# avianphysics/avian

Hardware: AMD Instinct MI355X
Metric: physics substeps/sec at N dynamic bodies (3D) (higher is better)
Workload: dtype f32; 1 GPU; cfg2_box_stack_100k; dynamic_bodies_per_gpu=100000, manifolds_per_gpu=678200, contact_points_per_gpu=2712800, broadphase_pairs=1244836, substeps=4, hip_graph=True, narrow_phase=out of path: fixed synthetic face manifolds

## Files before the change

### avian_amd/csrc/k_contacts.hip

```cpp
#include <cstdlib>

#include "avn_kernels.h"
#include "avn_body_ops.h"

namespace avn {

#define CONTACT_THREADS 64

template <class T> struct BodyRef {
    V3<T> v, om, dp;
    Q4<T> dq;
    V3<T> inv_mass;
    Sym3<T> I;
    T lin_w, ang_w;
};

template <class T> struct BodyView { Vec4<T> *lin, *ang, *dp, *dq, *sia, *sib; };
template <class T> __device__ __forceinline__ BodyView<T> global_bodies(const DW<T>& w) { return {w.sb_lin.p, w.sb_ang.p, w.sb_dp.p, w.sb_dq.p, w.si_a.p, w.si_b.p}; }

typedef uint32_t u32x4 __attribute__((ext_vector_type(4)));
#define AVN_BUF_AUX_SC1 16
template <class V> __device__ __forceinline__ __amdgpu_buffer_rsrc_t rec_rsrc(V* base) { return __builtin_amdgcn_make_buffer_rsrc((void*)base, 0, 0x7FFFFFFF, 0x00020000); }
__device__ __forceinline__ Vec4<float> ld_rec_agent(Vec4<float>* base, size_t idx) {
    const u32x4 r = __builtin_amdgcn_raw_buffer_load_b128(rec_rsrc(base), (int)(idx * sizeof(Vec4<float>)), 0, AVN_BUF_AUX_SC1);
    return make4<float>(__uint_as_float(r.x), __uint_as_float(r.y), __uint_as_float(r.z), __uint_as_float(r.w));
}
__device__ __forceinline__ Vec4<double> ld_rec_agent(Vec4<double>* base, size_t idx) {
    const __amdgpu_buffer_rsrc_t rs = rec_rsrc(base);
    const u32x4 a = __builtin_amdgcn_raw_buffer_load_b128(rs, (int)(idx * sizeof(Vec4<double>)), 0, AVN_BUF_AUX_SC1);
    const u32x4 b = __builtin_amdgcn_raw_buffer_load_b128(rs, (int)(idx * sizeof(Vec4<double>) + 16), 0, AVN_BUF_AUX_SC1);
    return make4<double>(__hiloint2double((int)a.y, (int)a.x), __hiloint2double((int)a.w, (int)a.z), __hiloint2double((int)b.y, (int)b.x), __hiloint2double((int)b.w, (int)b.z));
}
__device__ __forceinline__ void st_rec_agent(Vec4<float>* base, size_t idx, Vec4<float> v) {
    __builtin_amdgcn_raw_buffer_store_b128(u32x4{__float_as_uint(v.x), __float_as_uint(v.y), __float_as_uint(v.z), __float_as_uint(v.w)}, rec_rsrc(base), (int)(idx * sizeof(Vec4<float>)), 0,
                                           AVN_BUF_AUX_SC1);
}
__device__ __forceinline__ void st_rec_agent(Vec4<double>* base, size_t idx, Vec4<double> v) {
    const __amdgpu_buffer_rsrc_t rs = rec_rsrc(base);
    __builtin_amdgcn_raw_buffer_store_b128(u32x4{(uint32_t)__double2loint(v.x), (uint32_t)__double2hiint(v.x), (uint32_t)__double2loint(v.y), (uint32_t)__double2hiint(v.y)}, rs,
                                           (int)(idx * sizeof(Vec4<double>)), 0, AVN_BUF_AUX_SC1);
    __builtin_amdgcn_raw_buffer_store_b128(u32x4{(uint32_t)__double2loint(v.z), (uint32_t)__double2hiint(v.z), (uint32_t)__double2loint(v.w), (uint32_t)__double2hiint(v.w)}, rs,
                                           (int)(idx * sizeof(Vec4<double>) + 16), 0, AVN_BUF_AUX_SC1);
}
template <class T, bool WITH_DELTA> __device__ __forceinline__ void body_from_recs(Vec4<T> l, Vec4<T> a, Vec4<T> dp, Vec4<T> dq, Vec4<T> sa, Vec4<T> sb, bool no_body, bool dummy_inertia, BodyRef<T>& b) {
    const T z = T(0);
    b.v = V3<T>{no_body ? z : l.x, no_body ? z : l.y, no_body ? z : l.z};
    b.om = V3<T>{no_body ? z : a.x, no_body ? z : a.y, no_body ? z : a.z};
    b.lin_w = no_body ? z : l.w; b.ang_w = no_body ? z : a.w;
    const bool nd = no_body || !WITH_DELTA;
    b.dp = V3<T>{nd ? z : dp.x, nd ? z : dp.y, nd ? z : dp.z};
    b.dq = Q4<T>{nd ? z : dq.x, nd ? z : dq.y, nd ? z : dq.z, nd ? T(1) : dq.w};
    const bool ni = no_body || dummy_inertia;
    V3<T> em = effective_inv_mass<T>(sa.x, scalar_to_bits(sb.w));
    b.inv_mass = V3<T>{ni ? z : em.x, ni ? z : em.y, ni ? z : em.z};
    b.I = Sym3<T>{ni ? z : sa.y, ni ? z : sa.z, ni ? z : sa.w, ni ? z : sb.x, ni ? z : sb.y, ni ? z : sb.z};
}
template <class T, bool WITH_DELTA, int STRIDE, bool COH = false>
__device__ __forceinline__ void load_body(const BodyView<T>& bv, int idx, bool no_body, bool dummy_inertia, BodyRef<T>& b) {
    const size_t o = (size_t)idx * STRIDE;
    Vec4<T> l, a;
    if (COH) { l = ld_rec_agent(bv.lin, o); a = ld_rec_agent(bv.ang, o); }
    else { l = bv.lin[o]; a = bv.ang[o]; }
    Vec4<T> dp = make4<T>(0, 0, 0, 0), dq = make4<T>(0, 0, 0, 1);
    if (WITH_DELTA) { dp = bv.dp[o]; dq = bv.dq[o]; }
    Vec4<T> sa = bv.sia[o], sb = bv.sib[o];
    body_from_recs<T, WITH_DELTA>(l, a, dp, dq, sa, sb, no_body, dummy_inertia, b);
}
template <class T, int STRIDE, bool COH = false> __device__ __forceinline__ void store_body(const BodyView<T>& bv, int idx, bool no_body, const BodyRef<T>& b) {
    if (no_body) return;
    if (COH) { st_rec_agent(bv.lin, (size_t)idx * STRIDE, make4<T>(b.v, b.lin_w)); st_rec_agent(bv.ang, (size_t)idx * STRIDE, make4<T>(b.om, b.ang_w)); return; }
    bv.lin[(size_t)idx * STRIDE] = make4<T>(b.v, b.lin_w);
// ... 301 lines not shown
        contributions(r, ent, true, dl);
#pragma unroll
        for (uint32_t k = 0; k < AVN_MAX_MANIFOLD_POINTS; ++k) { v.x = v.x + dl.d[k][0]; v.y = v.y + dl.d[k][1]; v.z = v.z + dl.d[k][2]; om.x = om.x + dl.d[k][3]; om.y = om.y + dl.d[k][4]; om.z = om.z + dl.d[k][5]; }
    }
    const uint32_t n_ent = (uint32_t)__popc(mask);
    uint32_t rest = mask;
    for (uint32_t j0 = 0; j0 < n_ent; j0 += 4u) {
        uint32_t mine = rest;
        for (uint32_t t = 0; t < q; ++t) mine &= mine - 1u;
        const bool present = mine != 0u;
        const uint32_t c = present ? (uint32_t)__ffs((int)mine) - 1u : 0u;
        rest &= rest - 1u; rest &= rest - 1u; rest &= rest - 1u; rest &= rest - 1u;
        const uint32_t sc = present ? w.inc_slot[(size_t)c * w.inc_stride + body] : 0u;
        WarmRecords<T> r; QuadDelta<T> dl;
        warm_fetch<T>(w, sc, r);
        contributions(r, sc, present, dl);
        quad_accumulate<0, T>(dl, v, om); quad_accumulate<1, T>(dl, v, om); quad_accumulate<2, T>(dl, v, om); quad_accumulate<3, T>(dl, v, om);
    }
    if (q == 0u) {
        w.sb_lin[body] = make4<T>(v, l4.w);
        w.sb_ang[body] = make4<T>(om, a4.w);
    }
}

template <class T, int STRIDE>
__device__ __forceinline__ void warm_core(const DW<T>& w, const StepParams<T>& p, uint32_t m, const BodyView<T>& bv, int i1, int i2) {
    Vec4<T> h1 = w.c_h1[m], h0 = w.m_n[m];
    const uint32_t S = w.m_stride;
    Vec4<T> pa[AVN_MAX_MANIFOLD_POINTS], pb[AVN_MAX_MANIFOLD_POINTS], pd[AVN_MAX_MANIFOLD_POINTS];
#pragma unroll
    for (uint32_t k = 0; k < AVN_MAX_MANIFOLD_POINTS; ++k) { uint32_t s = k * S + m; pa[k] = w.c_pa[s]; pb[k] = w.c_pb[s]; pd[k] = w.c_pd[s]; }
    const uint32_t cm = scalar_to_bits(h1.w);
    const uint32_t np = cm & 7u;
    BodyRef<T> b1, b2;
    load_body<T, false, STRIDE>(bv, i1, cm & AVN_CM_NOBODY1, cm & AVN_CM_DOM1, b1);
    load_body<T, false, STRIDE>(bv, i2, cm & AVN_CM_NOBODY2, cm & AVN_CM_DOM2, b2);
    if (np == 0) return;
    const V3<T> normal = xyz<T>(h0);
    const V3<T> t0 = xyz<T>(h1), t1 = cross(t0, normal);
    const T coeff = p.warm_start_coefficient;
#pragma unroll
    for (uint32_t k = 0; k < AVN_MAX_MANIFOLD_POINTS; ++k) {
        if (k < np) {
            const Vec4<T> d = pd[k];
            const T tx = (cm & AVN_CM_TANGENT) ? d.z : T(0), ty = (cm & AVN_CM_TANGENT) ? d.w : T(0);
            const V3<T> imp = coeff * ((d.x * normal + tx * t0) + ty * t1);
            apply_impulse(b1, b2, imp, xyz<T>(pa[k]), xyz<T>(pb[k]));
        }
    }
    store_body<T, STRIDE>(bv, i1, cm & AVN_CM_NOBODY1, b1);
    store_body<T, STRIDE>(bv, i2, cm & AVN_CM_NOBODY2, b2);
}

template <class T, bool USE_BIAS, int STRIDE, bool COH = false>
__device__ __forceinline__ void solve_core(const DW<T>& w, const StepParams<T>& p, uint32_t m, const BodyView<T>& bv, int i1, int i2) {
    Vec4<T> h1 = w.c_h1[m];
    Vec4<T> h0 = w.m_n[m];
    Vec4<T> h2 = w.m_tv[m];
    uint32_t S = w.m_stride;
    Vec4<T> pa[AVN_MAX_MANIFOLD_POINTS], pb[AVN_MAX_MANIFOLD_POINTS], pc[AVN_MAX_MANIFOLD_POINTS], pd[AVN_MAX_MANIFOLD_POINTS];
#pragma unroll
    for (uint32_t k = 0; k < AVN_MAX_MANIFOLD_POINTS; ++k) {
        uint32_t s = k * S + m;
        pa[k] = w.c_pa[s]; pb[k] = w.c_pb[s]; pc[k] = w.c_pc[s]; pd[k] = w.c_pd[s];
    }
    uint32_t cm = scalar_to_bits(h1.w);
    uint32_t np = cm & 7u;
    BodyRef<T> b1, b2;
    load_body<T, true, STRIDE, COH>(bv, i1, cm & AVN_CM_NOBODY1, cm & AVN_CM_DOM1, b1);
    load_body<T, true, STRIDE, COH>(bv, i2, cm & AVN_CM_NOBODY2, cm & AVN_CM_DOM2, b2);
    if (np == 0) return;
    V3<T> normal = xyz<T>(h0);
    T friction = h0.w;
    SoftCoef<T> soft = (cm & AVN_CM_SOFT_ND) ? p.soft_non_dynamic : p.soft_dynamic;
    T delta_secs = p.h_adj;
    V3<T> delta_translation = b2.dp - b1.dp;
#pragma unroll
    for (uint32_t k = 0; k < AVN_MAX_MANIFOLD_POINTS; ++k) {
        if (k < np) {
            V3<T> a1 = xyz<T>(pa[k]), a2 = xyz<T>(pb[k]);
            V3<T> r1w = qrot(b1.dq, a1), r2w = qrot(b2.dq, a2);
            V3<T> delta_separation = delta_translation + (r2w - r1w);
            T separation = dot(delta_separation, normal) + pa[k].w;
            V3<T> relative_velocity = velocity_at_point(b2, a2) - velocity_at_point(b1, a1);
            T normal_speed = dot(relative_velocity, normal);
            T eff_mass = pb[k].w, acc = pd[k].x;
            T impulse;
            if (separation > T(0)) {
                impulse = -eff_mass * (normal_speed + separation / delta_secs);
            } else if (USE_BIAS) {
                T bias = smax(soft.bias * separation, -p.max_overlap_solve_speed);
                T scaled_mass = soft.mass_scale * eff_mass;
                T scaled_impulse = soft.impulse_scale * acc;
                impulse = -scaled_mass * (normal_speed + bias) - scaled_impulse;
            } else {
                impulse = -eff_mass * normal_speed;
            }
            T new_impulse = smax(acc + impulse, T(0));
            impulse = new_impulse - acc;
            pd[k].x = new_impulse;
            pd[k].y = pd[k].y + new_impulse;
            apply_impulse(b1, b2, impulse * normal, a1, a2);
        }
    }
    if (cm & AVN_CM_TANGENT) {
        V3<T> t0 = xyz<T>(h1), t1 = cross(t0, normal);
        V3<T> surface_velocity = xyz<T>(h2);
#pragma unroll
        for (uint32_t k = 0; k < AVN_MAX_MANIFOLD_POINTS; ++k) {
            if (k < np) {
                V3<T> a1 = xyz<T>(pa[k]), a2 = xyz<T>(pb[k]);
                V3<T> relative_velocity = velocity_at_point(b2, a2) - velocity_at_point(b1, a1);
                T impulse_limit = friction * pd[k].x;
                V3<T> rv = relative_velocity + surface_velocity;
                T ts1 = dot(rv, t0), ts2 = dot(rv, t1);
                T t11 = ts1 * ts1, t22 = ts2 * ts2, t12 = ts1 * ts2;
                T inv = t11 * pc[k].x + t22 * pc[k].y + t12 * pc[k].z;
                T effective_mass = (t11 + t22) * (T(1) / inv);
                if (finite_t(effective_mass)) {
                    V2<T> delta{effective_mass * ts1, effective_mass * ts2};
                    V2<T> ni = clamp_length_max(V2<T>{pd[k].z - delta.x, pd[k].w - delta.y}, impulse_limit);
                    V2<T> di{ni.x - pd[k].z, ni.y - pd[k].w};
                    pd[k].z = ni.x; pd[k].w = ni.y;
                    apply_impulse(b1, b2, di.x * t0 + di.y * t1, a1, a2);
                } else {
                    apply_impulse(b1, b2, vzero<T>(), a1, a2);
                }
            }
        }
    }
#pragma unroll
    for (uint32_t k = 0; k < AVN_MAX_MANIFOLD_POINTS; ++k)
        if (k < np) w.c_pd[k * S + m] = pd[k];
    store_body<T, STRIDE, COH>(bv, i1, cm & AVN_CM_NOBODY1, b1);
    store_body<T, STRIDE, COH>(bv, i2, cm & AVN_CM_NOBODY2, b2);
}

typedef float f2raw __attribute__((ext_vector_type(2)));
struct F2 {
    f2raw v;
    F2() = default;
    __device__ __forceinline__ F2(float a) : v{a, a} {}
    __device__ __forceinline__ F2(float lo, float hi) : v{lo, hi} {}
    __device__ __forceinline__ explicit F2(f2raw x) : v(x) {}
};
__device__ __forceinline__ F2 operator+(F2 a, F2 b) { return F2(a.v + b.v); }
__device__ __forceinline__ F2 operator-(F2 a, F2 b) { return F2(a.v - b.v); }
__device__ __forceinline__ F2 operator*(F2 a, F2 b) { return F2(a.v * b.v); }
__device__ __forceinline__ F2 operator-(F2 a) { return F2(-a.v); }
__device__ __forceinline__ F2 sub_lo_add_hi(F2 a, F2 b) {
    f2raw r;
    asm("v_pk_add_f32 %0, %1, %2 neg_lo:[0,1]" : "=v"(r) : "v"(a.v), "v"(b.v));
    return F2(r);
}
__device__ __forceinline__ V3<F2> sub_lo_add_hi(V3<F2> a, V3<F2> b) { return {sub_lo_add_hi(a.x, b.x), sub_lo_add_hi(a.y, b.y), sub_lo_add_hi(a.z, b.z)}; }
__device__ __forceinline__ V3<F2> pair3(V3<float> lo, V3<float> hi) { return {F2(lo.x, hi.x), F2(lo.y, hi.y), F2(lo.z, hi.z)}; }
__device__ __forceinline__ V3<F2> splat3(V3<float> a) { return {F2(a.x), F2(a.y), F2(a.z)}; }
__device__ __forceinline__ V3<float> lo3(V3<F2> a) { return {a.x.v.x, a.y.v.x, a.z.v.x}; }
__device__ __forceinline__ V3<float> hi3(V3<F2> a) { return {a.x.v.y, a.y.v.y, a.z.v.y}; }

struct BodyPair {
    V3<F2> v, om, inv_mass;
    Sym3<F2> I;
};
__device__ __forceinline__ void apply_impulse(BodyPair& b, V3<float> imp, V3<F2> anchors) {
    V3<F2> p = splat3(imp);
    b.v = sub_lo_add_hi(b.v, cmul(p, b.inv_mass));
    b.om = sub_lo_add_hi(b.om, smul(b.I, cross(anchors, p)));
}

struct NoPre { static constexpr bool on = false; };
struct FlowPre {
    static constexpr bool on = true;
    Vec4<float> h0, h1, h2, pa[AVN_MAX_MANIFOLD_POINTS], pb[AVN_MAX_MANIFOLD_POINTS], pc[AVN_MAX_MANIFOLD_POINTS], pd[AVN_MAX_MANIFOLD_POINTS];
    Vec4<float> l1, a1, dp1, dq1, sa1, sb1, l2, a2, dp2, dq2, sa2, sb2;
    bool no1, no2;
    uint32_t tag1, tag2;
};
template <bool USE_BIAS, int STRIDE, bool COH = false, class PRE = NoPre>
__device__ __forceinline__ void solve_core_packed(const DW<float>& w, const StepParams<float>& p, uint32_t m, const BodyView<float>& bv, int i1, int i2, const PRE& pre = PRE()) {
    typedef float T;
    Vec4<T> h1, h0, h2;
    uint32_t S = w.m_stride;
    Vec4<T> pa[AVN_MAX_MANIFOLD_POINTS], pb[AVN_MAX_MANIFOLD_POINTS], pc[AVN_MAX_MANIFOLD_POINTS], pd[AVN_MAX_MANIFOLD_POINTS];
    if constexpr (PRE::on) {
        h1 = pre.h1; h0 = pre.h0; h2 = pre.h2;
#pragma unroll
        for (uint32_t k = 0; k < AVN_MAX_MANIFOLD_POINTS; ++k) { pa[k] = pre.pa[k]; pb[k] = pre.pb[k]; pc[k] = pre.pc[k]; pd[k] = pre.pd[k]; }
    } else {
        h1 = w.c_h1[m];
        h0 = w.m_n[m];
        h2 = w.m_tv[m];
#pragma unroll
        for (uint32_t k = 0; k < AVN_MAX_MANIFOLD_POINTS; ++k) {
            uint32_t s = k * S + m;
            pa[k] = w.c_pa[s]; pb[k] = w.c_pb[s]; pc[k] = w.c_pc[s]; pd[k] = w.c_pd[s];
        }
    }
    uint32_t cm = scalar_to_bits(h1.w);
    uint32_t np = cm & 7u;
    BodyRef<T> b1, b2;
    bool no1 = cm & AVN_CM_NOBODY1, no2 = cm & AVN_CM_NOBODY2;
    if constexpr (PRE::on) {
        no1 = pre.no1; no2 = pre.no2;
        body_from_recs<T, true>(pre.l1, pre.a1, pre.dp1, pre.dq1, pre.sa1, pre.sb1, no1, cm & AVN_CM_DOM1, b1);
        body_from_recs<T, true>(pre.l2, pre.a2, pre.dp2, pre.dq2, pre.sa2, pre.sb2, no2, cm & AVN_CM_DOM2, b2);
        b1.lin_w = b1.ang_w = __uint_as_float(pre.tag1); b2.lin_w = b2.ang_w = __uint_as_float(pre.tag2);
        if (np == 0) {
            store_body<T, STRIDE, COH>(bv, i1, no1, b1);
            store_body<T, STRIDE, COH>(bv, i2, no2, b2);
            return;
        }
    } else {
        load_body<T, true, STRIDE, COH>(bv, i1, no1, cm & AVN_CM_DOM1, b1);
        load_body<T, true, STRIDE, COH>(bv, i2, no2, cm & AVN_CM_DOM2, b2);
        if (np == 0) return;
    }
    BodyPair bp;
    bp.v = pair3(b1.v, b2.v); bp.om = pair3(b1.om, b2.om); bp.inv_mass = pair3(b1.inv_mass, b2.inv_mass);
    bp.I = Sym3<F2>{F2(b1.I.m00, b2.I.m00), F2(b1.I.m01, b2.I.m01), F2(b1.I.m02, b2.I.m02), F2(b1.I.m11, b2.I.m11), F2(b1.I.m12, b2.I.m12), F2(b1.I.m22, b2.I.m22)};
    Q4<F2> dq{F2(b1.dq.x, b2.dq.x), F2(b1.dq.y, b2.dq.y), F2(b1.dq.z, b2.dq.z), F2(b1.dq.w, b2.dq.w)};
    V3<T> normal = xyz<T>(h0);
    T friction = h0.w;
    SoftCoef<T> soft = (cm & AVN_CM_SOFT_ND) ? p.soft_non_dynamic : p.soft_dynamic;
    T delta_secs = p.h_adj;
    V3<T> delta_translation = b2.dp - b1.dp;
#pragma unroll
    for (uint32_t k = 0; k < AVN_MAX_MANIFOLD_POINTS; ++k) {
        if (k < np) {
            V3<F2> anchors = pair3(xyz<T>(pa[k]), xyz<T>(pb[k]));
            V3<F2> rw = qrot(dq, anchors);
            V3<T> delta_separation = delta_translation + (hi3(rw) - lo3(rw));
            T separation = dot(delta_separation, normal) + pa[k].w;
            V3<F2> vap = bp.v + cross(bp.om, anchors);
            V3<T> relative_velocity = hi3(vap) - lo3(vap);
            T normal_speed = dot(relative_velocity, normal);
            T eff_mass = pb[k].w, acc = pd[k].x;
            T impulse;
            if (separation > T(0)) {
                impulse = -eff_mass * (normal_speed + separation / delta_secs);
            } else if (USE_BIAS) {
                T bias = smax(soft.bias * separation, -p.max_overlap_solve_speed);
                T scaled_mass = soft.mass_scale * eff_mass;
                T scaled_impulse = soft.impulse_scale * acc;
                impulse = -scaled_mass * (normal_speed + bias) - scaled_impulse;
            } else {
                impulse = -eff_mass * normal_speed;
            }
            T new_impulse = smax(acc + impulse, T(0));
            impulse = new_impulse - acc;
            pd[k].x = new_impulse;
            pd[k].y = pd[k].y + new_impulse;
            apply_impulse(bp, impulse * normal, anchors);
        }
    }
    if (cm & AVN_CM_TANGENT) {
        V3<T> t0 = xyz<T>(h1), t1 = cross(t0, normal);
        V3<T> surface_velocity = xyz<T>(h2);
#pragma unroll
        for (uint32_t k = 0; k < AVN_MAX_MANIFOLD_POINTS; ++k) {
            if (k < np) {
                V3<F2> anchors = pair3(xyz<T>(pa[k]), xyz<T>(pb[k]));
                V3<F2> vap = bp.v + cross(bp.om, anchors);
                V3<T> relative_velocity = hi3(vap) - lo3(vap);
                T impulse_limit = friction * pd[k].x;
                V3<T> rv = relative_velocity + surface_velocity;
                T ts1 = dot(rv, t0), ts2 = dot(rv, t1);
                T t11 = ts1 * ts1, t22 = ts2 * ts2, t12 = ts1 * ts2;
                T inv = t11 * pc[k].x + t22 * pc[k].y + t12 * pc[k].z;
                T effective_mass = (t11 + t22) * (T(1) / inv);
                if (finite_t(effective_mass)) {
                    V2<T> delta{effective_mass * ts1, effective_mass * ts2};
                    V2<T> ni = clamp_length_max(V2<T>{pd[k].z - delta.x, pd[k].w - delta.y}, impulse_limit);
                    V2<T> di{ni.x - pd[k].z, ni.y - pd[k].w};
                    pd[k].z = ni.x; pd[k].w = ni.y;
                    apply_impulse(bp, di.x * t0 + di.y * t1, anchors);
                } else {
                    apply_impulse(bp, vzero<T>(), anchors);
                }
            }
        }
    }
#pragma unroll
    for (uint32_t k = 0; k < AVN_MAX_MANIFOLD_POINTS; ++k)
        if (k < np) w.c_pd[k * S + m] = pd[k];
    b1.v = lo3(bp.v); b1.om = lo3(bp.om); b2.v = hi3(bp.v); b2.om = hi3(bp.om);
    store_body<T, STRIDE, COH>(bv, i1, no1, b1);
    store_body<T, STRIDE, COH>(bv, i2, no2, b2);
}
template <class T, bool USE_BIAS, int STRIDE, bool COH = false> struct SolveDispatch {
    static __device__ __forceinline__ void run(const DW<T>& w, const StepParams<T>& p, uint32_t m, const BodyView<T>& bv, int i1, int i2) { solve_core<T, USE_BIAS, STRIDE, COH>(w, p, m, bv, i1, i2); }
};
template <bool USE_BIAS, int STRIDE, bool COH> struct SolveDispatch<float, USE_BIAS, STRIDE, COH> {
    static __device__ __forceinline__ void run(const DW<float>& w, const StepParams<float>& p, uint32_t m, const BodyView<float>& bv, int i1, int i2) { solve_core_packed<USE_BIAS, STRIDE, COH>(w, p, m, bv, i1, i2); }
};

namespace oct {
template <int CTRL> __device__ __forceinline__ float dpp(float x) { return __int_as_float(__builtin_amdgcn_update_dpp(0, __float_as_int(x), CTRL, 0xF, 0xF, true)); }
__device__ __forceinline__ float rot1(float x) { return dpp<0xC9>(x); }
__device__ __forceinline__ float rot2(float x) { return dpp<0xD2>(x); }
__device__ __forceinline__ float bx(float x) { return dpp<0x00>(x); }
__device__ __forceinline__ float by(float x) { return dpp<0x55>(x); }
__device__ __forceinline__ float bz(float x) { return dpp<0xAA>(x); }
__device__ __forceinline__ float partner(float x) {
    int t = __builtin_amdgcn_update_dpp(0, __float_as_int(x), 0x104 , 0xF, 0x5, false);
    t = __builtin_amdgcn_update_dpp(t, __float_as_int(x), 0x114 , 0xF, 0xA, false);
    return __int_as_float(t);
}
__device__ __forceinline__ float dot3(float a, float b) { const float p = a * b; return (bx(p) + by(p)) + bz(p); }
}

#define OCT_MANIFOLDS_PER_WAVE 8
template <bool USE_BIAS>
__device__ __forceinline__ void solve_core_oct(const DW<float>& w, const StepParams<float>& p, uint32_t m, uint32_t lane8) {
    using namespace oct;
    const uint32_t j = lane8 & 3u;
    const bool q = (lane8 & 4u) != 0u;
    auto sel = [&](float x, float y, float z) { return j == 0u ? x : (j == 1u ? y : z); };
    const Vec4<float> h1 = w.c_h1[m], h0 = w.m_n[m], h2 = w.m_tv[m];
    const uint32_t S = w.m_stride;
    Vec4<float> pa[AVN_MAX_MANIFOLD_POINTS], pb[AVN_MAX_MANIFOLD_POINTS], pc[AVN_MAX_MANIFOLD_POINTS], pd[AVN_MAX_MANIFOLD_POINTS];
#pragma unroll
    for (uint32_t k = 0; k < AVN_MAX_MANIFOLD_POINTS; ++k) {
        const uint32_t s = k * S + m;
        pa[k] = w.c_pa[s]; pb[k] = w.c_pb[s]; pc[k] = w.c_pc[s]; pd[k] = w.c_pd[s];
    }
    const int2 bi = w.m_bodies[m];
    const uint32_t cm = scalar_to_bits(h1.w);
    const uint32_t np = cm & 7u;
    const size_t o = (size_t)(q ? bi.y : bi.x);
    const Vec4<float> l4 = w.sb_lin[o], a4 = w.sb_ang[o], dp4 = w.sb_dp[o], dq4 = w.sb_dq[o], sa = w.si_a[o], sb = w.si_b[o];
    if (np == 0) return;
    const bool no_body = cm & (q ? AVN_CM_NOBODY2 : AVN_CM_NOBODY1);
    const bool ni = no_body || (cm & (q ? AVN_CM_DOM2 : AVN_CM_DOM1));
    float v0 = no_body ? 0.0f : sel(l4.x, l4.y, l4.z);
    float om0 = no_body ? 0.0f : sel(a4.x, a4.y, a4.z);
    const float dpj = no_body ? 0.0f : sel(dp4.x, dp4.y, dp4.z);
    const float b0 = no_body ? 0.0f : sel(dq4.x, dq4.y, dq4.z);
    const float qw = no_body ? 1.0f : dq4.w;
    const V3<float> em = effective_inv_mass<float>(sa.x, scalar_to_bits(sb.w));
    const float im = ni ? 0.0f : sel(em.x, em.y, em.z);
    const float I0 = ni ? 0.0f : sel(sa.y, sa.z, sa.w), I1 = ni ? 0.0f : sel(sa.z, sb.x, sb.y), I2 = ni ? 0.0f : sel(sa.w, sb.y, sb.z);
    const uint32_t neg = q ? 0u : 0x80000000u;
    auto signed_for_body = [&](float x) { return __uint_as_float(__float_as_uint(x) ^ neg); };
    auto d21 = [&](float x) {
        float r;
        asm("s_nop 1\n\tv_sub_f32_dpp %0, %1, %1 row_shl:4 row_mask:0xf bank_mask:0x5\n\tv_subrev_f32_dpp %0, %1, %1 row_shr:4 row_mask:0xf bank_mask:0xa" : "=&v"(r) : "v"(x));
// ... 133 lines not shown
    V3<T> normal = xyz<T>(w.m_n[m]);
    BodyRef<T> b1, b2;
    load_body<T, false, STRIDE, COH>(bv, i1, cm & AVN_CM_NOBODY1, cm & AVN_CM_DOM1, b1);
    load_body<T, false, STRIDE, COH>(bv, i2, cm & AVN_CM_NOBODY2, cm & AVN_CM_DOM2, b2);
    restitution_chain<T>(w, p, m, np, restitution, normal, b1, b2);
    store_body<T, STRIDE, COH>(bv, i1, cm & AVN_CM_NOBODY1, b1);
    store_body<T, STRIDE, COH>(bv, i2, cm & AVN_CM_NOBODY2, b2);
}

template <class T, int STRIDE>
__device__ __forceinline__ void skeleton_core(const DW<T>& w, uint32_t m, const BodyView<T>& bv, int i1, int i2) {
    Vec4<T> h1 = w.c_h1[m];
    Vec4<T> h0 = w.m_n[m];
    Vec4<T> h2 = w.m_tv[m];
    uint32_t S = w.m_stride;
    Vec4<T> pa[AVN_MAX_MANIFOLD_POINTS], pb[AVN_MAX_MANIFOLD_POINTS], pc[AVN_MAX_MANIFOLD_POINTS], pd[AVN_MAX_MANIFOLD_POINTS];
#pragma unroll
    for (uint32_t k = 0; k < AVN_MAX_MANIFOLD_POINTS; ++k) {
        uint32_t s = k * S + m;
        pa[k] = w.c_pa[s]; pb[k] = w.c_pb[s]; pc[k] = w.c_pc[s]; pd[k] = w.c_pd[s];
    }
    uint32_t cm = scalar_to_bits(h1.w);
    uint32_t np = cm & 7u;
    BodyRef<T> b1, b2;
    load_body<T, true, STRIDE>(bv, i1, cm & AVN_CM_NOBODY1, cm & AVN_CM_DOM1, b1);
    load_body<T, true, STRIDE>(bv, i2, cm & AVN_CM_NOBODY2, cm & AVN_CM_DOM2, b2);
    if (np == 0) return;
    T acc = ((h0.x + h0.y) + (h0.z + h0.w)) + ((h2.x + h2.y) + (h2.z + h2.w)) + ((h1.x + h1.y) + h1.z);
#pragma unroll
    for (uint32_t k = 0; k < AVN_MAX_MANIFOLD_POINTS; ++k)
        acc = acc + (((pa[k].x + pa[k].y) + (pa[k].z + pa[k].w)) + ((pb[k].x + pb[k].y) + (pb[k].z + pb[k].w)) + ((pc[k].x + pc[k].y) + (pc[k].z + pc[k].w)));
    acc = acc + (dot(b1.dp, b2.dp) + dot(b1.inv_mass, b2.inv_mass)) + ((b1.dq.x + b1.dq.y) + (b1.dq.z + b1.dq.w)) + ((b2.dq.x + b2.dq.y) + (b2.dq.z + b2.dq.w));
    acc = acc + ((b1.I.m00 + b1.I.m01) + (b1.I.m02 + b1.I.m11) + (b1.I.m12 + b1.I.m22)) + ((b2.I.m00 + b2.I.m01) + (b2.I.m02 + b2.I.m11) + (b2.I.m12 + b2.I.m22));
    const bool never = scalar_to_bits(acc) == 0x7FC12345u;
#pragma unroll
    for (uint32_t k = 0; k < AVN_MAX_MANIFOLD_POINTS; ++k)
        if (k < np) { if (never) pd[k].y = acc; w.c_pd[k * S + m] = pd[k]; }
    if (never) { b1.v.x = acc; b2.om.x = acc; }
    store_body<T, STRIDE>(bv, i1, cm & AVN_CM_NOBODY1, b1);
    store_body<T, STRIDE>(bv, i2, cm & AVN_CM_NOBODY2, b2);
}

enum { PASS_WARM = 0, PASS_BIAS = 1, PASS_RELAX = 2, PASS_RESTITUTION = 3, PASS_SKELETON = 5 };
template <class T, int PASS, bool COH = false> __device__ __forceinline__ void pass_one(const DW<T>& w, const StepParams<T>& p, uint32_t m) {
    const int2 b = w.m_bodies[m];
    const BodyView<T> bv = global_bodies(w);
    if (PASS == PASS_WARM) warm_core<T, 2>(w, p, m, bv, b.x, b.y);
    else if (PASS == PASS_SKELETON) skeleton_core<T, 2>(w, m, bv, b.x, b.y);
    else if (PASS == PASS_BIAS) SolveDispatch<T, true, 2, COH>::run(w, p, m, bv, b.x, b.y);
    else if (PASS == PASS_RELAX) SolveDispatch<T, false, 2, COH>::run(w, p, m, bv, b.x, b.y);
    else restitution_core<T, 2, COH>(w, p, m, bv, b.x, b.y);
}

template <class T, int PASS>
__global__ __launch_bounds__(CONTACT_THREADS) void k_color_pass(DW<T> w, StepParams<T> p, uint32_t color, uint32_t arg_base, uint32_t arg_end) {
    uint32_t base = arg_base, end = arg_end;
    if (arg_end == 0u) { base = w.color_offsets[color]; end = w.color_offsets[color + 1]; }
    const uint32_t tiles = (end - base + CONTACT_THREADS - 1u) / CONTACT_THREADS, per = (tiles + 7u) >> 3, row = blockIdx.x >> 3;
    if (row >= per) return;
    const uint32_t blk = (blockIdx.x & 7u) * per + row;
    uint32_t m = base + blk * CONTACT_THREADS + threadIdx.x;
    if (m >= end) return;
    pass_one<T, PASS>(w, p, m);
}
#define OVERFLOW_THREADS 256
template <class T, int PASS>
__global__ __launch_bounds__(OVERFLOW_THREADS) void k_overflow_pass(DW<T> w, StepParams<T> p, const uint32_t* __restrict__ comp_level_begin,
                                                                    const uint32_t* __restrict__ level_offsets, const uint32_t* __restrict__ order) {
    const uint32_t c = blockIdx.x;
    const uint32_t l0 = comp_level_begin[c], l1 = comp_level_begin[c + 1];
    for (uint32_t l = l0; l < l1; ++l) {
        const uint32_t k0 = level_offsets[l], k1 = level_offsets[l + 1];
        for (uint32_t k = k0 + threadIdx.x; k < k1; k += OVERFLOW_THREADS) pass_one<T, PASS>(w, p, order[k]);
        __syncthreads();
    }
}

template <class T, int PASS>
__global__ __launch_bounds__(CONTACT_THREADS) void k_overflow_flow(DW<T> w, StepParams<T> p, OverflowFlow of, uint32_t epoch) {
    __shared__ uint32_t s_tile;
    const uint32_t lane = threadIdx.x;
    if (lane == 0) s_tile = atomicAdd(&of.tiles[epoch], 1u);
    __syncthreads();
    const uint32_t o0 = w.color_offsets[AVN_COLOR_OVERFLOW_INDEX], n23 = w.color_offsets[AVN_COLOR_OVERFLOW_INDEX + 1] - o0;
    const uint32_t i = s_tile * CONTACT_THREADS + lane;
    const bool valid = i < n23;
    const uint32_t m = o0 + (valid ? i : 0u);
    uint32_t r1 = 0xFFFFFFFFu, r2 = 0xFFFFFFFFu, t1 = 0, t2 = 0;
    int2 b = make_int2(0, 0);
    if (valid) {
        b = w.m_bodies[m];
        r1 = of.rank[2 * i]; r2 = of.rank[2 * i + 1];
        if (r1 != 0xFFFFFFFFu) t1 = epoch * (w.inc_off[b.x + 1] - w.inc_off[b.x]) + r1;
        if (r2 != 0xFFFFFFFFu) t2 = epoch * (w.inc_off[b.y + 1] - w.inc_off[b.y]) + r2;
    }
    bool done = !valid;
    for (uint32_t it = 0;; ++it) {
        if (!done) {
            const bool ready = (r1 == 0xFFFFFFFFu || __hip_atomic_load(&of.ticket[b.x], __ATOMIC_RELAXED, __HIP_MEMORY_SCOPE_AGENT) == t1) &&
                               (r2 == 0xFFFFFFFFu || __hip_atomic_load(&of.ticket[b.y], __ATOMIC_RELAXED, __HIP_MEMORY_SCOPE_AGENT) == t2);
            if (ready) {
                asm volatile("" ::: "memory");
                pass_one<T, PASS, true>(w, p, m);
                asm volatile("s_waitcnt vmcnt(0)" ::: "memory");
                if (r1 != 0xFFFFFFFFu) __hip_atomic_fetch_add(&of.ticket[b.x], 1u, __ATOMIC_RELAXED, __HIP_MEMORY_SCOPE_AGENT);
                if (r2 != 0xFFFFFFFFu && !(r1 != 0xFFFFFFFFu && b.x == b.y)) __hip_atomic_fetch_add(&of.ticket[b.y], 1u, __ATOMIC_RELAXED, __HIP_MEMORY_SCOPE_AGENT);
                done = true;
            }
        }
        if (__all(done)) break;
        if (it > (1u << 20)) { if (lane == 0) atomicOr(of.error, 2u); break; }
        __builtin_amdgcn_s_sleep(8);
    }
}
#define OVF_TAG_SHIFT 20
template <int PASS>
// ... 126 lines not shown
template <class T> void launch_prepare_contact_constraints(const DW<T>& w, const StepParams<T>& p, hipStream_t s, bool count_clean, const RowsView<T>* rows, bool lazy) {
    if (!count_clean) (void)hipMemsetAsync(w.constraint_count, 0, sizeof(uint32_t), s);
    if (!w.n_manifolds) return;
    static const bool pa_always = avn_env("AVN_PREP_WRITE_PA") != nullptr;
    const dim3 grid(prepare_grid_blocks(w.n_manifolds));
    if (rows) hipLaunchKernelGGL((k_prepare_contact_constraints<T, true>), dim3(prepare_grid_blocks(w.n_manifolds)), dim3(PREP_TILE), 0, s, w, p, *rows);
    else if (lazy && !pa_always) hipLaunchKernelGGL((k_prepare_contact_constraints<T, false, true, true>), grid, dim3(PREP_TILE), 0, s, w, p, RowsView<T>{});
    else if (lazy) hipLaunchKernelGGL((k_prepare_contact_constraints<T, false, true, false>), grid, dim3(PREP_TILE), 0, s, w, p, RowsView<T>{});
    else if (!pa_always) hipLaunchKernelGGL((k_prepare_contact_constraints<T, false, false, true>), grid, dim3(PREP_TILE), 0, s, w, p, RowsView<T>{});
    else hipLaunchKernelGGL((k_prepare_contact_constraints<T, false>), dim3(prepare_grid_blocks(w.n_manifolds)), dim3(PREP_TILE), 0, s, w, p, RowsView<T>{});
}
template <class T> void launch_store_contact_impulses(const DW<T>& w, hipStream_t s) {
    if (w.n_manifolds) hipLaunchKernelGGL(k_store_contact_impulses<T>, dim3((w.n_manifolds + 255) / 256), dim3(256), 0, s, w);
}
uint32_t color_grid_blocks(uint32_t count) {
    uint32_t nb = (count + CONTACT_THREADS - 1) / CONTACT_THREADS;
    return ((nb + 7u) / 8u) * 8u;
}
template <class T, int PASS>
__global__ __launch_bounds__(CONTACT_THREADS) void k_overflow_level(DW<T> w, StepParams<T> p, const uint32_t* __restrict__ order, uint32_t first, uint32_t count) {
    uint32_t i = xcd_block(blockIdx.x, gridDim.x) * CONTACT_THREADS + threadIdx.x;
    if (i >= count) return;
    pass_one<T, PASS>(w, p, order[first + i]);
}
template <class T, int PASS> struct OctLaunch { static bool run(const DW<T>&, const StepParams<T>&, uint32_t, uint32_t, uint32_t, uint32_t, hipStream_t) { return false; } };
template <int PASS> struct OctLaunch<float, PASS> {
    static bool run(const DW<float>& w, const StepParams<float>& p, uint32_t c, uint32_t blocks, uint32_t b, uint32_t e, hipStream_t s) {
        if constexpr (PASS == PASS_BIAS || PASS == PASS_RELAX) {
            hipLaunchKernelGGL((k_color_pass_oct<PASS>), dim3(blocks * (CONTACT_THREADS / OCT_MANIFOLDS_PER_WAVE)), dim3(CONTACT_THREADS), 0, s, w, p, c, b, e);
            return true;
        }
        return false;
    }
};
template <class T, int PASS> static uint32_t launch_pass(const DW<T>& w, const StepParams<T>& p, const uint32_t* grid_blocks, const uint32_t* arg_offsets, const OverflowSchedule& ovf, hipStream_t s, uint32_t oct_mask,
                                                         avn_solver_forms* forms) {
    uint32_t launches = 0;
    constexpr bool loop_pass = PASS != PASS_RESTITUTION;
    if (grid_blocks[AVN_COLOR_OVERFLOW_INDEX] && ovf.n_glevels) {
        uint32_t largest = 0;
        for (uint32_t l = 0; l < ovf.n_glevels; ++l) {
            uint32_t first = ovf.glevel_offsets[l], count = ovf.glevel_offsets[l + 1] - first;
            if (!count) continue;
            hipLaunchKernelGGL((k_overflow_level<T, PASS>), dim3(color_grid_blocks(count)), dim3(CONTACT_THREADS), 0, s, w, p, ovf.gorder, first, count);
            ++launches;
            if (color_grid_blocks(count) > largest) largest = color_grid_blocks(count);
        }
        if (forms && loop_pass) { forms->overflow_form = AVN_OVERFLOW_FORM_LEVEL; forms->overflow_components = 0; forms->overflow_levels = launches; forms->overflow_grid_blocks = largest; }
    } else if (grid_blocks[AVN_COLOR_OVERFLOW_INDEX] && ovf.n_components) {
        hipLaunchKernelGGL((k_overflow_pass<T, PASS>), dim3(ovf.n_components), dim3(OVERFLOW_THREADS), 0, s, w, p, ovf.comp_level_begin, ovf.level_offsets, ovf.order);
        ++launches;
        if (forms && loop_pass) { forms->overflow_form = AVN_OVERFLOW_FORM_COMPONENT; forms->overflow_components = ovf.n_components; forms->overflow_levels = 0; forms->overflow_grid_blocks = ovf.n_components; }
    }
    for (uint32_t c = 0; c < AVN_COLOR_OVERFLOW_INDEX; ++c)
        if (grid_blocks[c]) {
            uint32_t b = arg_offsets ? arg_offsets[c] : 0u, e = arg_offsets ? arg_offsets[c + 1] : 0u;
            if (arg_offsets && e == b) continue;
            uint32_t form = AVN_COLOUR_FORM_OCT;
            if (!((oct_mask >> c) & 1u) || !OctLaunch<T, PASS>::run(w, p, c, grid_blocks[c], b, e, s)) {
                hipLaunchKernelGGL((k_color_pass<T, PASS>), dim3(grid_blocks[c]), dim3(CONTACT_THREADS), 0, s, w, p, c, b, e);
                form = AVN_COLOUR_FORM_LANE;
            }
            ++launches;
            if (forms && loop_pass) { forms->colour_form[c] = form; forms->colour_grid_blocks[c] = grid_blocks[c]; forms->colour_ranges_from = arg_offsets ? AVN_RANGES_FROM_ARGUMENTS : AVN_RANGES_FROM_DEVICE; }
            else if (forms) forms->restitution_colour_form[c] = form;
        }
    return launches;
}
template <class T>
__global__ __launch_bounds__(256) void k_build_incidence_slots(DW<T> w) {
    uint32_t m = blockIdx.x * 256 + threadIdx.x;
    if (m >= w.color_offsets[AVN_COLOR_OVERFLOW_INDEX]) return;
    uint32_t lo = 0, hi = AVN_COLOR_OVERFLOW_INDEX;
    while (hi - lo > 1) { uint32_t mid = (lo + hi) >> 1; if (w.color_offsets[mid] <= m) lo = mid; else hi = mid; }
    int2 b = w.m_bodies[m];
    w.inc_slot[(size_t)lo * w.inc_stride + (uint32_t)b.x] = m;
    w.inc_slot[(size_t)lo * w.inc_stride + (uint32_t)b.y] = m | 0x80000000u;
}
template <class T> void launch_build_incidence_slots(const DW<T>& w, hipStream_t s, bool cleared) {
    if (!cleared) (void)hipMemsetAsync(w.inc_slot, 0xFF, (size_t)AVN_COLOR_OVERFLOW_INDEX * w.inc_stride * sizeof(uint32_t), s);
    if (w.n_manifolds) hipLaunchKernelGGL(k_build_incidence_slots<T>, dim3((w.n_manifolds + 255) / 256), dim3(256), 0, s, w);
}
template <class T, int PASS, bool CACHE>
__device__ __forceinline__ void island_colours(const DW<T>& w, const StepParams<T>& p, const uint2* ent, uint32_t e0, const BodyView<T>& bv, const uint32_t* col) {
    const uint32_t t = threadIdx.x;
    for (uint32_t c = 0; c < AVN_GRAPH_COLOR_COUNT; ++c) {
        const uint32_t begin = col[c], end = col[c + 1];
        if (begin == end) continue;
        const bool serial = c == 0;
        for (uint32_t e = begin + (serial ? 0u : t); e < end; e += serial ? 1u : ISLAND_THREADS) {
            if (serial && t != 0) continue;
            const uint2 en = ent[CACHE ? e - e0 : e];
            const uint32_t m = CACHE ? e - e0 : en.x;
            const int i1 = (int)(en.y & 0xFFFFu), i2 = (int)(en.y >> 16);
            if (PASS == PASS_WARM) warm_core<T, 1>(w, p, m, bv, i1, i2);
            else if (PASS == PASS_BIAS) SolveDispatch<T, true, 1>::run(w, p, m, bv, i1, i2);
            else SolveDispatch<T, false, 1>::run(w, p, m, bv, i1, i2);
        }
        __syncthreads();
    }
}
template <class T, bool CACHE>
__global__ __launch_bounds__(ISLAND_THREADS) void k_island_substeps(DW<T> w, StepParams<T> p, IslandBlocks ib, uint32_t substeps, uint32_t iterations) {
    __shared__ Vec4<T> lds[ISLAND_LDS_VEC4];
    __shared__ uint32_t l_col[AVN_GRAPH_COLOR_COUNT + 1];
    const uint32_t t = threadIdx.x, blk = blockIdx.x;
    const uint32_t b0 = ib.body_off[blk], nb = ib.body_off[blk + 1] - b0;
    const uint32_t nbmax = CACHE ? ib.max_bodies : ISLAND_MAX_BODIES, LM = ib.max_manifolds;
    Vec4<T>* const l_lin = lds, *const l_ang = lds + nbmax, *const l_dp = lds + 2 * nbmax, *const l_dq = lds + 3 * nbmax, *const l_sia = lds + 4 * nbmax,
                   *const l_sib = lds + 5 * nbmax;
    Vec4<T>* const R = lds + 6 * nbmax;
    if (t <= AVN_GRAPH_COLOR_COUNT) l_col[t] = ib.col_off[(size_t)blk * AVN_GRAPH_COLOR_COUNT + t];
    for (uint32_t l = t; l < nb; l += ISLAND_THREADS) {
// ... 103 lines not shown
```

Measured before the change: 2906 substeps/s.

## Pass compact kernel args and prefetch all solve inputs up front in lane color pass

For bias and relax passes, the lane color kernel now receives a compact SolveArgs struct holding only the pointers and params the solver needs, instead of the full DW and StepParams. The offsets are read through the constant address space and the args are pinned in scalar registers. A new lane_pass issues all manifold, contact-point and body loads before any compute, with compiler fences to keep that order, then hands the preloaded records to the solve core through a new LanePre path. The aim is smaller kernel-argument traffic and more memory-level parallelism, at the cost of higher register pressure from holding every record live at once.

```diff
diff --git a/avian_amd/csrc/k_contacts.hip b/avian_amd/csrc/k_contacts.hip
--- a/avian_amd/csrc/k_contacts.hip
+++ b/avian_amd/csrc/k_contacts.hip
@@ -17,6 +17,23 @@
 
 template <class T> struct BodyView { Vec4<T> *lin, *ang, *dp, *dq, *sia, *sib; };
 template <class T> __device__ __forceinline__ BodyView<T> global_bodies(const DW<T>& w) { return {w.sb_lin.p, w.sb_ang.p, w.sb_dp.p, w.sb_dq.p, w.si_a.p, w.si_b.p}; }
+
+template <class T> struct SolveArgs {
+    using V = Vec4<T>;
+    int2* m_bodies;
+    V *c_h1, *m_n, *m_tv, *c_pa, *c_pb, *c_pc, *c_pd;
+    Pair2<V> sb_lin, sb_ang, sb_dp, sb_dq, si_a, si_b;
+    uint32_t* color_offsets;
+    uint32_t m_stride;
+    SoftCoef<T> soft_dynamic, soft_non_dynamic;
+    T h_adj, max_overlap_solve_speed;
+    SolveArgs() = default;
+    SolveArgs(const DW<T>& w, const StepParams<T>& p)
+        : m_bodies(w.m_bodies), c_h1(w.c_h1), m_n(w.m_n), m_tv(w.m_tv), c_pa(w.c_pa), c_pb(w.c_pb), c_pc(w.c_pc), c_pd(w.c_pd), sb_lin(w.sb_lin), sb_ang(w.sb_ang), sb_dp(w.sb_dp),
+          sb_dq(w.sb_dq), si_a(w.si_a), si_b(w.si_b), color_offsets(w.color_offsets), m_stride(w.m_stride), soft_dynamic(p.soft_dynamic), soft_non_dynamic(p.soft_non_dynamic), h_adj(p.h_adj),
+          max_overlap_solve_speed(p.max_overlap_solve_speed) {}
+};
+template <class T> __device__ __forceinline__ BodyView<T> global_bodies(const SolveArgs<T>& w) { return {w.sb_lin.p, w.sb_ang.p, w.sb_dp.p, w.sb_dq.p, w.si_a.p, w.si_b.p}; }
 
 typedef uint32_t u32x4 __attribute__((ext_vector_type(4)));
 #define AVN_BUF_AUX_SC1 16
@@ -424,23 +441,42 @@
     store_body<T, STRIDE>(bv, i2, cm & AVN_CM_NOBODY2, b2);
 }
 
-template <class T, bool USE_BIAS, int STRIDE, bool COH = false>
-__device__ __forceinline__ void solve_core(const DW<T>& w, const StepParams<T>& p, uint32_t m, const BodyView<T>& bv, int i1, int i2) {
-    Vec4<T> h1 = w.c_h1[m];
-    Vec4<T> h0 = w.m_n[m];
-    Vec4<T> h2 = w.m_tv[m];
+struct NoPre { static constexpr bool on = false, flow = false; };
+template <class T> struct LanePre {
+    static constexpr bool on = true, flow = false;
+    Vec4<T> h0, h1, h2, pa[AVN_MAX_MANIFOLD_POINTS], pb[AVN_MAX_MANIFOLD_POINTS], pc[AVN_MAX_MANIFOLD_POINTS], pd[AVN_MAX_MANIFOLD_POINTS];
+    Vec4<T> l1, a1, dp1, dq1, sa1, sb1, l2, a2, dp2, dq2, sa2, sb2;
+};
+
+template <class T, bool USE_BIAS, int STRIDE, bool COH = false, class PRE = NoPre, class W = DW<T>, class P = StepParams<T>>
+__device__ __forceinline__ void solve_core(const W& w, const P& p, uint32_t m, const BodyView<T>& bv, int i1, int i2, const PRE& pre = PRE()) {
+    Vec4<T> h1, h0, h2;
     uint32_t S = w.m_stride;
     Vec4<T> pa[AVN_MAX_MANIFOLD_POINTS], pb[AVN_MAX_MANIFOLD_POINTS], pc[AVN_MAX_MANIFOLD_POINTS], pd[AVN_MAX_MANIFOLD_POINTS];
-#pragma unroll
-    for (uint32_t k = 0; k < AVN_MAX_MANIFOLD_POINTS; ++k) {
-        uint32_t s = k * S + m;
-        pa[k] = w.c_pa[s]; pb[k] = w.c_pb[s]; pc[k] = w.c_pc[s]; pd[k] = w.c_pd[s];
+    if constexpr (PRE::on) {
+        h1 = pre.h1; h0 = pre.h0; h2 = pre.h2;
+#pragma unroll
+        for (uint32_t k = 0; k < AVN_MAX_MANIFOLD_POINTS; ++k) { pa[k] = pre.pa[k]; pb[k] = pre.pb[k]; pc[k] = pre.pc[k]; pd[k] = pre.pd[k]; }
+    } else {
+        h1 = w.c_h1[m];
+        h0 = w.m_n[m];
+        h2 = w.m_tv[m];
+#pragma unroll
+        for (uint32_t k = 0; k < AVN_MAX_MANIFOLD_POINTS; ++k) {
+            uint32_t s = k * S + m;
+            pa[k] = w.c_pa[s]; pb[k] = w.c_pb[s]; pc[k] = w.c_pc[s]; pd[k] = w.c_pd[s];
+        }
     }
     uint32_t cm = scalar_to_bits(h1.w);
     uint32_t np = cm & 7u;
     BodyRef<T> b1, b2;
-    load_body<T, true, STRIDE, COH>(bv, i1, cm & AVN_CM_NOBODY1, cm & AVN_CM_DOM1, b1);
-    load_body<T, true, STRIDE, COH>(bv, i2, cm & AVN_CM_NOBODY2, cm & AVN_CM_DOM2, b2);
+    if constexpr (PRE::on) {
+        body_from_recs<T, true>(pre.l1, pre.a1, pre.dp1, pre.dq1, pre.sa1, pre.sb1, cm & AVN_CM_NOBODY1, cm & AVN_CM_DOM1, b1);
+        body_from_recs<T, true>(pre.l2, pre.a2, pre.dp2, pre.dq2, pre.sa2, pre.sb2, cm & AVN_CM_NOBODY2, cm & AVN_CM_DOM2, b2);
+    } else {
+        load_body<T, true, STRIDE, COH>(bv, i1, cm & AVN_CM_NOBODY1, cm & AVN_CM_DOM1, b1);
+        load_body<T, true, STRIDE, COH>(bv, i2, cm & AVN_CM_NOBODY2, cm & AVN_CM_DOM2, b2);
+    }
     if (np == 0) return;
     V3<T> normal = xyz<T>(h0);
     T friction = h0.w;
@@ -541,16 +577,15 @@
     b.om = sub_lo_add_hi(b.om, smul(b.I, cross(anchors, p)));
 }
 
-struct NoPre { static constexpr bool on = false; };
 struct FlowPre {
-    static constexpr bool on = true;
+    static constexpr bool on = true, flow = true;
     Vec4<float> h0, h1, h2, pa[AVN_MAX_MANIFOLD_POINTS], pb[AVN_MAX_MANIFOLD_POINTS], pc[AVN_MAX_MANIFOLD_POINTS], pd[AVN_MAX_MANIFOLD_POINTS];
     Vec4<float> l1, a1, dp1, dq1, sa1, sb1, l2, a2, dp2, dq2, sa2, sb2;
     bool no1, no2;
     uint32_t tag1, tag2;
 };
-template <bool USE_BIAS, int STRIDE, bool COH = false, class PRE = NoPre>
-__device__ __forceinline__ void solve_core_packed(const DW<float>& w, const StepParams<float>& p, uint32_t m, const BodyView<float>& bv, int i1, int i2, const PRE& pre = PRE()) {
+template <bool USE_BIAS, int STRIDE, bool COH = false, class PRE = NoPre, class W = DW<float>, class P = StepParams<float>>
+__device__ __forceinline__ void solve_core_packed(const W& w, const P& p, uint32_t m, const BodyView<float>& bv, int i1, int i2, const PRE& pre = PRE()) {
     typedef float T;
     Vec4<T> h1, h0, h2;
     uint32_t S = w.m_stride;
@@ -573,7 +608,7 @@
     uint32_t np = cm & 7u;
     BodyRef<T> b1, b2;
     bool no1 = cm & AVN_CM_NOBODY1, no2 = cm & AVN_CM_NOBODY2;
-    if constexpr (PRE::on) {
+    if constexpr (PRE::flow) {
         no1 = pre.no1; no2 = pre.no2;
         body_from_recs<T, true>(pre.l1, pre.a1, pre.dp1, pre.dq1, pre.sa1, pre.sb1, no1, cm & AVN_CM_DOM1, b1);
         body_from_recs<T, true>(pre.l2, pre.a2, pre.dp2, pre.dq2, pre.sa2, pre.sb2, no2, cm & AVN_CM_DOM2, b2);
@@ -583,6 +618,10 @@
             store_body<T, STRIDE, COH>(bv, i2, no2, b2);
             return;
         }
+    } else if constexpr (PRE::on) {
+        body_from_recs<T, true>(pre.l1, pre.a1, pre.dp1, pre.dq1, pre.sa1, pre.sb1, no1, cm & AVN_CM_DOM1, b1);
+        body_from_recs<T, true>(pre.l2, pre.a2, pre.dp2, pre.dq2, pre.sa2, pre.sb2, no2, cm & AVN_CM_DOM2, b2);
+        if (np == 0) return;
     } else {
         load_body<T, true, STRIDE, COH>(bv, i1, no1, cm & AVN_CM_DOM1, b1);
         load_body<T, true, STRIDE, COH>(bv, i2, no2, cm & AVN_CM_DOM2, b2);
@@ -661,10 +700,14 @@
     store_body<T, STRIDE, COH>(bv, i2, no2, b2);
 }
 template <class T, bool USE_BIAS, int STRIDE, bool COH = false> struct SolveDispatch {
-    static __device__ __forceinline__ void run(const DW<T>& w, const StepParams<T>& p, uint32_t m, const BodyView<T>& bv, int i1, int i2) { solve_core<T, USE_BIAS, STRIDE, COH>(w, p, m, bv, i1, i2); }
+    template <class W, class P, class PRE = NoPre> static __device__ __forceinline__ void run(const W& w, const P& p, uint32_t m, const BodyView<T>& bv, int i1, int i2, const PRE& pre = PRE()) {
+        solve_core<T, USE_BIAS, STRIDE, COH, PRE>(w, p, m, bv, i1, i2, pre);
+    }
 };
 template <bool USE_BIAS, int STRIDE, bool COH> struct SolveDispatch<float, USE_BIAS, STRIDE, COH> {
-    static __device__ __forceinline__ void run(const DW<float>& w, const StepParams<float>& p, uint32_t m, const BodyView<float>& bv, int i1, int i2) { solve_core_packed<USE_BIAS, STRIDE, COH>(w, p, m, bv, i1, i2); }
+    template <class W, class P, class PRE = NoPre> static __device__ __forceinline__ void run(const W& w, const P& p, uint32_t m, const BodyView<float>& bv, int i1, int i2, const PRE& pre = PRE()) {
+        solve_core_packed<USE_BIAS, STRIDE, COH, PRE>(w, p, m, bv, i1, i2, pre);
+    }
 };
 
 namespace oct {
@@ -904,16 +947,63 @@
     else restitution_core<T, 2, COH>(w, p, m, bv, b.x, b.y);
 }
 
+#define AVN_LOAD_FENCE() asm volatile("" ::: "memory")
+template <class T, int PASS> __device__ __forceinline__ void lane_pass(const SolveArgs<T>& a, uint32_t m) {
+    LanePre<T> r;
+    const int2 b = a.m_bodies[m];
+    r.h1 = a.c_h1[m];
+    r.h0 = a.m_n[m];
+    r.h2 = a.m_tv[m];
+    AVN_LOAD_FENCE();
+    if ((scalar_to_bits(r.h1.w) & 7u) == 0u) return;
+    const size_t o1 = (size_t)b.x, o2 = (size_t)b.y;
+    r.dq1 = a.sb_dq[o1]; r.dq2 = a.sb_dq[o2]; r.dp1 = a.sb_dp[o1]; r.dp2 = a.sb_dp[o2];
+    r.l1 = a.sb_lin[o1]; r.l2 = a.sb_lin[o2]; r.a1 = a.sb_ang[o1]; r.a2 = a.sb_ang[o2];
+    r.sa1 = a.si_a[o1]; r.sa2 = a.si_a[o2]; r.sb1 = a.si_b[o1]; r.sb2 = a.si_b[o2];
+    AVN_LOAD_FENCE();
+    const uint32_t S = a.m_stride;
+#pragma unroll
+    for (uint32_t k = 0; k < AVN_MAX_MANIFOLD_POINTS; ++k) {
+        const uint32_t s = k * S + m;
+        r.pa[k] = a.c_pa[s]; r.pb[k] = a.c_pb[s]; r.pd[k] = a.c_pd[s];
+        AVN_LOAD_FENCE();
+    }
+#pragma unroll
+    for (uint32_t k = 0; k < AVN_MAX_MANIFOLD_POINTS; ++k) r.pc[k] = a.c_pc[k * S + m];
+    AVN_LOAD_FENCE();
+    SolveDispatch<T, PASS == PASS_BIAS, 2, false>::run(a, a, m, global_bodies(a), b.x, b.y, r);
+}
+template <class T> __device__ __forceinline__ void hold_args(const SolveArgs<T>& a) {
+    asm volatile("" ::"s"(a.m_bodies), "s"(a.c_h1), "s"(a.m_n), "s"(a.m_tv), "s"(a.c_pa), "s"(a.c_pb), "s"(a.c_pc), "s"(a.c_pd), "s"(a.sb_lin.p), "s"(a.sb_ang.p), "s"(a.sb_dp.p), "s"(a.sb_dq.p),
+                 "s"(a.si_a.p), "s"(a.si_b.p), "s"(a.m_stride), "s"(a.soft_dynamic.bias), "s"(a.soft_dynamic.mass_scale), "s"(a.soft_dynamic.impulse_scale), "s"(a.soft_non_dynamic.bias),
+                 "s"(a.soft_non_dynamic.mass_scale), "s"(a.soft_non_dynamic.impulse_scale), "s"(a.h_adj), "s"(a.max_overlap_solve_speed));
+}
+template <class T> struct WideArgs {
+    DW<T> w; StepParams<T> p;
+    WideArgs(const DW<T>& w_, const StepParams<T>& p_) : w(w_), p(p_) {}
+};
+typedef const uint32_t __attribute__((address_space(4))) * ConstWords;
+template <class T> __device__ __forceinline__ void live_range(const WideArgs<T>& a, uint32_t color, uint32_t& base, uint32_t& end) { base = a.w.color_offsets[color]; end = a.w.color_offsets[color + 1]; }
+template <class T> __device__ __forceinline__ void live_range(const SolveArgs<T>& a, uint32_t color, uint32_t& base, uint32_t& end) {
+    const ConstWords offs = (ConstWords)(uintptr_t)a.color_offsets;
+    base = offs[color]; end = offs[color + 1];
+}
+template <class T, int PASS> struct ColorArgs : WideArgs<T> { using WideArgs<T>::WideArgs; };
+template <class T> struct ColorArgs<T, PASS_BIAS> : SolveArgs<T> { using SolveArgs<T>::SolveArgs; };
+template <class T> struct ColorArgs<T, PASS_RELAX> : SolveArgs<T> { using SolveArgs<T>::SolveArgs; };
+template <class T, int PASS> __device__ __forceinline__ void color_one(const WideArgs<T>& a, uint32_t m) { pass_one<T, PASS>(a.w, a.p, m); }
+template <class T, int PASS> __device__ __forceinline__ void color_one(const SolveArgs<T>& a, uint32_t m) { lane_pass<T, PASS>(a, m); }
 template <class T, int PASS>
-__global__ __launch_bounds__(CONTACT_THREADS) void k_color_pass(DW<T> w, StepParams<T> p, uint32_t color, uint32_t arg_base, uint32_t arg_end) {
+__global__ __launch_bounds__(CONTACT_THREADS) void k_color_pass(ColorArgs<T, PASS> a, uint32_t color, uint32_t arg_base, uint32_t arg_end) {
+    if constexpr (PASS == PASS_BIAS || PASS == PASS_RELAX) hold_args(a);
     uint32_t base = arg_base, end = arg_end;
-    if (arg_end == 0u) { base = w.color_offsets[color]; end = w.color_offsets[color + 1]; }
+    if (arg_end == 0u) live_range(a, color, base, end);
     const uint32_t tiles = (end - base + CONTACT_THREADS - 1u) / CONTACT_THREADS, per = (tiles + 7u) >> 3, row = blockIdx.x >> 3;
     if (row >= per) return;
     const uint32_t blk = (blockIdx.x & 7u) * per + row;
     uint32_t m = base + blk * CONTACT_THREADS + threadIdx.x;
     if (m >= end) return;
-    pass_one<T, PASS>(w, p, m);
+    color_one<T, PASS>(a, m);
 }
 #define OVERFLOW_THREADS 256
 template <class T, int PASS>
@@ -1146,13 +1236,14 @@
         ++launches;
         if (forms && loop_pass) { forms->overflow_form = AVN_OVERFLOW_FORM_COMPONENT; forms->overflow_components = ovf.n_components; forms->overflow_levels = 0; forms->overflow_grid_blocks = ovf.n_components; }
     }
+    const ColorArgs<T, PASS> args(w, p);
     for (uint32_t c = 0; c < AVN_COLOR_OVERFLOW_INDEX; ++c)
         if (grid_blocks[c]) {
             uint32_t b = arg_offsets ? arg_offsets[c] : 0u, e = arg_offsets ? arg_offsets[c + 1] : 0u;
             if (arg_offsets && e == b) continue;
             uint32_t form = AVN_COLOUR_FORM_OCT;
             if (!((oct_mask >> c) & 1u) || !OctLaunch<T, PASS>::run(w, p, c, grid_blocks[c], b, e, s)) {
-                hipLaunchKernelGGL((k_color_pass<T, PASS>), dim3(grid_blocks[c]), dim3(CONTACT_THREADS), 0, s, w, p, c, b, e);
+                hipLaunchKernelGGL((k_color_pass<T, PASS>), dim3(grid_blocks[c]), dim3(CONTACT_THREADS), 0, s, args, c, b, e);
                 form = AVN_COLOUR_FORM_LANE;
             }
             ++launches;
```

New measurement: 3159 substeps/s (median of 6 runs). 8.7% higher.
